# sjulier/Refactored_ORB_SLAM2

Hardware: AMD Instinct MI355X
Metric: frames/s (extract+match) at KITTI 1241×376, 2000 feat; 1/2/4/8 GPU + CPU ref (higher is better)
Workload: dtype u8; 1 GPU; kitti_stereo_1241x376_2000feat_8lvl: 2x ORBextractor + ComputeStereoMatches + SearchByProjection(cur,last); parallelism=frame-shard x1, collective=none, driver=torch, queries=one pass: orbfe_track_queries_stereo_device

## Files before the change

refactored_orb_slam2_amd/csrc/extract_kernels.hip:

```cpp
#include <stdlib.h>
#include <string.h>

#include "orbfe_internal.h"
#include "../../include/orb_pattern_data.h"

#define WAVE 64

__device__ __forceinline__ int wave_incl_scan(int v) {
  v += __builtin_amdgcn_update_dpp(0, v, 0x111, 0xf, 0xf, false);
  v += __builtin_amdgcn_update_dpp(0, v, 0x112, 0xf, 0xf, false);
  v += __builtin_amdgcn_update_dpp(0, v, 0x114, 0xf, 0xf, false);
  v += __builtin_amdgcn_update_dpp(0, v, 0x118, 0xf, 0xf, false);
  v += __builtin_amdgcn_update_dpp(0, v, 0x142, 0xa, 0xf, false);
  v += __builtin_amdgcn_update_dpp(0, v, 0x143, 0xc, 0xf, false);
  return v;
}

template <int T>
__device__ __forceinline__ int block_incl_scan_t(int v, int* tmp, int* total) {
  const int tid = threadIdx.x;
  const int lane = tid & (WAVE - 1), wid = tid >> 6;
  int s = wave_incl_scan(v);
  if (T == WAVE) {
    *total = __builtin_amdgcn_readlane(s, WAVE - 1);
    return s;
  }
  __syncthreads();
  if (lane == WAVE - 1) tmp[wid] = s;
  __syncthreads();
  int off = 0, tot = 0;
#pragma unroll
  for (int i = 0; i < T / WAVE; i++) {
    int t = tmp[i];
    if (i < wid) off += t;
    tot += t;
  }
  *total = tot;
  return s + off;
}

template <int T>
__device__ __forceinline__ int block_incl_scan_alt(int v, int* tmp, int& slot, int* total) {
  const int tid = threadIdx.x;
  const int lane = tid & (WAVE - 1), wid = tid >> 6;
  const int s = wave_incl_scan(v);
  int* t = tmp + slot * (T / WAVE);
  slot ^= 1;
  if (lane == WAVE - 1) t[wid] = s;
  __syncthreads();
  int off = 0, tot = 0;
#pragma unroll
  for (int i = 0; i < T / WAVE; i++) {
    const int x = t[i];
    if (i < wid) off += x;
    tot += x;
  }
  *total = tot;
  return s + off;
}

__device__ __forceinline__ int reflect101(int p, int len) {
  if (len == 1) return 0;
  while (p < 0 || p >= len) p = (p < 0) ? -p : 2 * (len - 1) - p;
  return p;
}

__global__ __launch_bounds__(256) void copy_level0_kernel(const uint8_t* __restrict__ src, int sstride,
                                                           unsigned long long simg, uint8_t* __restrict__ dst,
                                                           int dpitch, unsigned long long dimg, int w, int h, int tiled) {
  const int nchunk = (w + 15) >> 4;
  const int item = blockIdx.x * 256 + threadIdx.x;
  const int y = (int)((item + 0.5f) * (1.0f / (float)nchunk));
  const int x16 = (item - y * nchunk) * 16;
  if (y >= h) return;
  const uint8_t* S = src + (size_t)blockIdx.z * simg + (size_t)y * sstride;
  uint32_t out[4];
  if (x16 + 20 <= w) {
    const uintptr_t A = reinterpret_cast<uintptr_t>(S + x16);
    const uint32_t sh = (uint32_t)(A & 3);
    const uint32_t* B = reinterpret_cast<const uint32_t*>(A - sh);
    uint32_t d[5];
#pragma unroll
    for (int i = 0; i < 5; i++) d[i] = B[i];
#pragma unroll
// ... 1394 lines not shown
  hi = (int)__builtin_amdgcn_perm(t23, t01, 0x07060302u);
}
#ifndef BT_MFMA
#define BT_MFMA 1
#endif
#define BT_W 64
#define BT_H ORBFE_BLUR_TILE_H
#if BT_MFMA
#define BT_INP 96
#define BT_COL0 12
#else
#define BT_INP 80
#define BT_COL0 0
#endif
#define BT_HP 68
#ifndef BT_NT_STORE
#define BT_NT_STORE 1
#endif
#ifndef BT_NT_LOAD
#define BT_NT_LOAD 0
#endif
#ifndef BT_XCD_IMAGES
#define BT_XCD_IMAGES 1
#endif
#ifndef BT_SCALAR_TILE
#define BT_SCALAR_TILE 1
#endif
#ifndef BT_MIN_WAVES
#define BT_MIN_WAVES 2
#endif
#ifndef BT_THREADS
#define BT_THREADS 128
#endif
template <bool RESIZE, int THREADS>
__global__ __launch_bounds__(THREADS, BT_MIN_WAVES) void blur_level_kernel(PyrView src, PyrView dst, const BlurTile* __restrict__ tiles, int n_tiles,
                                                         LevelResize rz) {
#if BT_MFMA
  __shared__ __attribute__((aligned(16))) uint8_t in[65 * BT_INP];
#else
  __shared__ __attribute__((aligned(16))) uint8_t in[(BT_H + 6) * BT_INP];
  __shared__ __attribute__((aligned(16))) uint32_t hbp[((BT_H + 6) / 2) * BT_HP];
#endif
  const int tid = threadIdx.x;
#if BT_MFMA
  const int mlane = tid & 63, mwave = __builtin_amdgcn_readfirstlane(tid >> 6);
  const v4i* mtab = reinterpret_cast<const v4i*>(g_blur_tile_tab);
  const v4i HB = mtab[mlane];
#endif
#if BT_XCD_IMAGES
  int tile_id = (int)blockIdx.x, img = (int)blockIdx.y;
  {
    const unsigned gx = gridDim.x;
    const unsigned lin = blockIdx.y * gx + blockIdx.x;
    const unsigned grp = lin / (8u * gx);
    if (8u * grp + 8u <= gridDim.y) {
      const unsigned within = lin - grp * 8u * gx;
      img = (int)(8u * grp + (within & 7u));
      tile_id = (int)(within >> 3);
    }
  }
#else
  const int q = blockIdx.x >> 3, img = (int)blockIdx.y;
  const int tile_id = (int)blockIdx.x >= (n_tiles / 64) * 64 ? (int)blockIdx.x : (q >> 3) * 64 + (blockIdx.x & 7) * 8 + (q & 7);
#endif
#if BT_SCALAR_TILE
  static_assert(sizeof(BlurTile) == 16, "four dwords");
  BlurTile t;
  {
    const __attribute__((address_space(4))) uint32_t* q =
        (const __attribute__((address_space(4))) uint32_t*)(uintptr_t)(tiles + __builtin_amdgcn_readfirstlane(tile_id));
    uint32_t w4[4];
#pragma unroll
    for (int j = 0; j < 4; j++) w4[j] = q[j];
    __builtin_memcpy(&t, w4, sizeof(t));
  }
#else
  const BlurTile t = tiles[tile_id];
#endif
  const int lvl = t.level;
  const int w = src.w[lvl], h = src.h[lvl], pitch = src.pitch[lvl];
  const uint8_t* S = src.base[lvl] + (size_t)img * src.img_stride[lvl];
  uint8_t* D = const_cast<uint8_t*>(dst.base[lvl]) + (size_t)img * dst.img_stride[lvl];
  const int ox = t.tx * BT_W, oy = t.ty * BT_H;
  const bool stiled = (src.tiled >> lvl) & 1u;
  const int J = t.j0 + (tid & (ORBFE_FUSE_DWORDS - 1));
  __shared__ uint4 ytap[16 * ORBFE_FUSE_ROWS];
  __shared__ uint32_t ydst[16 * ORBFE_FUSE_ROWS];
  uint2 txr[4], tyl = make_uint2(0u, 0u);
  if constexpr (RESIZE) {
#pragma unroll
    for (int i = 0; i < 4; i++) txr[i] = reinterpret_cast<const uint2*>(rz.xt)[min(4 * J + i, rz.dw - 1)];
    tyl = reinterpret_cast<const uint2*>(rz.yt)[min(t.r0 + min(tid, 16 * ORBFE_FUSE_ROWS - 1), rz.dh - 1)];
  }
  {
    uint32_t* in32 = reinterpret_cast<uint32_t*>(in);
    constexpr int NC = RESIZE ? 19 : 18;
    constexpr int RPP = THREADS / NC, NLD = (BT_H + 6 + RPP - 1) / RPP;
    const int r0 = tid / NC, c = tid - r0 * NC;
    const int x = ox - 4 + 4 * c;
    uint32_t v[NLD];
    const bool interior = oy >= 3 && oy + BT_H + 3 <= h && ox >= 4 && ox - 4 + 4 * NC <= w;
    const bool tilepath = stiled && BT_COL0 != 0;
    if (r0 < RPP && !tilepath) {
      if (interior && stiled) {
        const uint32_t xoff = ((uint32_t)(x >> 4) << 7) + (uint32_t)(x & 15), tstep = (uint32_t)(pitch >> 4) << 7;
#pragma unroll
        for (int k = 0; k < NLD; k++) {
          const int y = oy - 3 + r0 + RPP * k;
          v[k] = r0 + RPP * k < BT_H + 6 ? *reinterpret_cast<const uint32_t*>(S + (uint32_t)(y >> 3) * tstep + (uint32_t)((y & 7) * 16) + xoff) : 0u;
        }
      } else if (interior) {
        const uint8_t* p0 = S + (size_t)(oy - 3 + r0) * pitch + x;
#pragma unroll
        for (int k = 0; k < NLD; k++)
#if BT_NT_LOAD
          v[k] = r0 + RPP * k < BT_H + 6 ? __builtin_nontemporal_load(reinterpret_cast<const uint32_t*>(p0 + (size_t)(RPP * k) * pitch)) : 0u;
#else
          v[k] = r0 + RPP * k < BT_H + 6 ? *reinterpret_cast<const uint32_t*>(p0 + (size_t)(RPP * k) * pitch) : 0u;
#endif
      } else {
        const bool whole = x >= 0 && x + 3 < w;
        int gx[4];
#pragma unroll
        for (int j = 0; j < 4; j++) gx[j] = reflect101(x + j, w);
#pragma unroll
        for (int k = 0; k < NLD; k++) {
          const int r = r0 + RPP * k;
          v[k] = 0u;
          if (r < BT_H + 6) {
            const int yy = reflect101(oy + r - 3, h);
            auto px = [&](int xx) { return (uint32_t)S[orbfe_level_offset(xx, yy, pitch, stiled)]; };
            if (whole) v[k] = *reinterpret_cast<const uint32_t*>(S + orbfe_level_offset(x, yy, pitch, stiled));
            else v[k] = px(gx[0]) | (px(gx[1]) << 8) | (px(gx[2]) << 16) | (px(gx[3]) << 24);
          }
        }
      }
#pragma unroll
      for (int k = 0; k < NLD; k++) {
        const int r = r0 + RPP * k;
        if (r < BT_H + 6) in32[r * (BT_INP / 4) + BT_COL0 / 4 + c] = v[k];
      }
    }
#if BT_MFMA
    if (tilepath) {
      constexpr int N_TOP = 3 * 6, N_MID = 7 * 8 * 6, N_ALL = N_TOP + N_MID + 3 * 6;
      constexpr int NP = (N_ALL + THREADS - 1) / THREADS;
      const int ty0 = (oy - 3) >> 3, tx0 = (ox - 16) >> 4;
      const int tiles_y = (h + 7) >> 3, tiles_x = pitch >> 4;
      const uint32_t tstep = (uint32_t)tiles_x << 7;
      auto piece = [&](int pid, int& tyi, int& txi, int& rr) {
        if (pid < N_TOP) { txi = (pid * 43) >> 7; rr = 5 + pid - 3 * txi; tyi = 0; }
        else if (pid < N_TOP + N_MID) { const int q = pid - N_TOP, tl = q >> 3; rr = q & 7; tyi = (tl * 43) >> 8; txi = tl - 6 * tyi; tyi += 1; }
        else { const int q = pid - N_TOP - N_MID; txi = (q * 43) >> 7; rr = q - 3 * txi; tyi = 8; }
      };
      uint4 pv[NP];
      uint32_t lds_at[NP];
#pragma unroll
      for (int k = 0; k < NP; k++) {
        int tyi, txi, rr;
        piece(min(tid + k * THREADS, N_ALL - 1), tyi, txi, rr);
        const int tr = min(max(ty0 + tyi, 0), tiles_y - 1), tc = min(max(tx0 + txi, 0), tiles_x - 1);
        pv[k] = *reinterpret_cast<const uint4*>(S + (uint32_t)tr * tstep + ((uint32_t)tc << 7) + (uint32_t)(rr * 16));
        lds_at[k] = (uint32_t)((tyi * 8 + rr - 5) * BT_INP + 16 * txi);
      }
#pragma unroll
      for (int k = 0; k < NP; k++)
        if (tid + k * THREADS < N_ALL) *reinterpret_cast<uint4*>(in + lds_at[k]) = pv[k];
      if (!interior) {
        __syncthreads();
        {
          const int nl = ox == 0 ? 3 : 0, nr = w < ox - 4 + 4 * NC ? 3 : 0;
          for (int i = tid; i < (BT_H + 6) * (nl + nr); i += THREADS) {
            const int wr = (int)((i + 0.5f) * (1.0f / (float)(nl + nr))), j = i - wr * (nl + nr);
            const int xx = j < nl ? j - 3 : w + (j - nl);
            const int y = oy - 3 + wr;
            if (y >= 0 && y < h && xx - (ox - 16) < BT_INP)
              in[wr * BT_INP + (xx - (ox - 16))] = in[wr * BT_INP + (reflect101(xx, w) - (ox - 16))];
          }
        }
        __syncthreads();
        {
          const int nt = oy == 0 ? 3 : 0, nb = h < oy + BT_H + 3 ? 3 : 0;
          for (int i = tid; i < (nt + nb) * (BT_INP / 4); i += THREADS) {
            const int j = (int)((i + 0.5f) * (1.0f / (float)(BT_INP / 4))), cdw = i - j * (BT_INP / 4);
            const int y = j < nt ? j - 3 : h + (j - nt);
            const int wr = y - (oy - 3), ws = reflect101(y, h) - (oy - 3);
            if (wr >= 0 && wr < BT_H + 6) in32[wr * (BT_INP / 4) + cdw] = in32[ws * (BT_INP / 4) + cdw];
          }
        }
      }
    }
#endif
  }
  if constexpr (RESIZE)
    if (tid < 16 * ORBFE_FUSE_ROWS) {
      const int ra = (int)(int16_t)(tyl.x & 0xffff) - (oy - 3), rb = (int)(int16_t)(tyl.x >> 16) - (oy - 3);
      ytap[tid] = make_uint4((uint32_t)(ra * BT_INP), (uint32_t)(rb * BT_INP), (tyl.y & 0xffffu) << 12, (tyl.y >> 16) << 12);
      const int yd = t.r0 + tid;
      ydst[tid] = rz.dst_tiled ? (uint32_t)(yd >> 3) * ((uint32_t)(rz.dpitch >> 4) << 7) + (uint32_t)((yd & 7) * 16) : (uint32_t)yd * (uint32_t)rz.dpitch;
    }
  __syncthreads();
  if constexpr (RESIZE) {
    typedef __attribute__((ext_vector_type(2))) unsigned short us2;
    if (J < t.j1) {
      const int s00 = (int)(int16_t)(txr[0].x & 0xffff);
      const int base = s00 - (ox - 4) + BT_COL0;
      const uint32_t sh = (uint32_t)base & 3u;
      uint32_t sel[4], cp[4];
#pragma unroll
      for (int i = 0; i < 4; i++) {
        const uint32_t o = (uint32_t)((int)(int16_t)(txr[i].x & 0xffff) - s00);
        sel[i] = o | 0x0c000c00u | ((o + 1) << 16);
        cp[i] = txr[i].y;
      }
      const uint32_t trow = (uint32_t)(uintptr_t)(in + (base & ~3));
      auto hrow2 = [&](uint32_t off_a, uint32_t off_b, uint32_t (&ha)[4], uint32_t (&hb)[4]) {
        unsigned long long a01, b01;
        uint32_t a2, b2;
        asm volatile("ds_read2_b32 %0, %4 offset1:1\n\t"
                     "ds_read_b32 %1, %4 offset:8\n\t"
                     "ds_read2_b32 %2, %5 offset1:1\n\t"
                     "ds_read_b32 %3, %5 offset:8\n\t"
                     "s_waitcnt lgkmcnt(0)"
                     : "=&v"(a01), "=&v"(a2), "=&v"(b01), "=&v"(b2)
                     : "v"(trow + off_a), "v"(trow + off_b)
                     : "memory");
        const uint32_t A0 = __builtin_amdgcn_alignbyte((uint32_t)(a01 >> 32), (uint32_t)a01, sh), A1 = __builtin_amdgcn_alignbyte(a2, (uint32_t)(a01 >> 32), sh);
        const uint32_t B0w = __builtin_amdgcn_alignbyte((uint32_t)(b01 >> 32), (uint32_t)b01, sh), B1w = __builtin_amdgcn_alignbyte(b2, (uint32_t)(b01 >> 32), sh);
#pragma unroll
        for (int i = 0; i < 4; i++) {
          const uint32_t ua = __builtin_amdgcn_perm(A1, A0, sel[i]), ub = __builtin_amdgcn_perm(B1w, B0w, sel[i]);
          ha[i] = __builtin_amdgcn_udot2(__builtin_bit_cast(us2, ua), __builtin_bit_cast(us2, cp[i]), 0u, false) & ~15u;
          hb[i] = __builtin_amdgcn_udot2(__builtin_bit_cast(us2, ub), __builtin_bit_cast(us2, cp[i]), 0u, false) & ~15u;
        }
      };
      uint8_t* Nimg = rz.dst + (size_t)img * rz.dimg;
      const uint32_t ncol = rz.dst_tiled ? (((uint32_t)((4 * J) >> 4) << 7) + (uint32_t)((4 * J) & 15)) : (uint32_t)(4 * J);
      for (int yi = tid >> 4; yi < t.r1 - t.r0; yi += THREADS / 16) {
        uint8_t* N = Nimg + (ncol + ydst[yi]);
        {
          const uint4 ty = ytap[yi];
          uint32_t h0[4], h1[4];
          hrow2(ty.x, ty.y, h0, h1);
          const uint32_t B0 = ty.z, B1 = ty.w;
          uint32_t sm[4];
#pragma unroll
          for (int i = 0; i < 4; i++) sm[i] = mulhi_u24(B0, h0[i]) + mulhi_u24(B1, h1[i]) + 2u;
          const uint32_t P01 = (sm[0] | (sm[1] << 16)) >> 2, P23 = (sm[2] | (sm[3] << 16)) >> 2;
          *reinterpret_cast<uint32_t*>(N) = __builtin_amdgcn_perm(P23, P01, 0x06040200u);
        }
      }
    }
  }
#if BT_MFMA
  {
    const int q = mlane >> 4, r = mlane & 15;
    const v4i c128 = {128, 128, 128, 128}, zero = {0, 0, 0, 0};
    const v4i cfin = {8388608 + 32768, 8388608 + 32768, 8388608 + 32768, 8388608 + 32768};
    v4i TB[4];
#pragma unroll
    for (int b = 0; b < 4; b++) TB[b] = mtab[(1 + b) * 64 + mlane];
    const uint32_t bstep = (uint32_t)(dst.pitch[lvl] >> 4) << 8;
#pragma unroll
    for (int g = mwave; g < BT_W / 16; g += THREADS / 64) {
      v4i Xh, Xl;
      {
        const v4i* arow = reinterpret_cast<const v4i*>(in + r * BT_INP + 16 * g + 16 * q);
        v4i A[4];
#pragma unroll
        for (int blk = 0; blk < 4; blk++) A[blk] = arow[blk * BT_INP];
        int ph[4], pl[4];
#pragma unroll
        for (int blk = 0; blk < 4; blk++) {
          const v4i d = __builtin_amdgcn_mfma_i32_16x16x64_i8(A[blk] ^ (int)0x80808080, HB, c128, 0, 0, 0);
          blur_pack(d, ph[blk], pl[blk]);
        }
        Xh = v4i{ph[0], ph[1], ph[2], ph[3]};
        Xl = v4i{pl[0], pl[1], pl[2], pl[3]};
      }
      const int gx = ox + 16 * g + 4 * q;
      uint8_t* o = D + blur_tiled_offset(gx, oy + r, dst.pitch[lvl]);
#pragma unroll
      for (int b = 0; b < 4; b++) {
        const v4i vh = __builtin_amdgcn_mfma_i32_16x16x64_i8(Xh, TB[b], zero, 0, 0, 0);
        const v4i vl = __builtin_amdgcn_mfma_i32_16x16x64_i8(Xl, TB[b], cfin, 0, 0, 0);
        const uint32_t r0 = ((uint32_t)vh.x << 8) + (uint32_t)vl.x, r1 = ((uint32_t)vh.y << 8) + (uint32_t)vl.y;
        const uint32_t r2 = ((uint32_t)vh.z << 8) + (uint32_t)vl.z, r3 = ((uint32_t)vh.w << 8) + (uint32_t)vl.w;
        const uint32_t out = __builtin_amdgcn_perm(r1, r0, 0x0c0c0602u) | __builtin_amdgcn_perm(r3, r2, 0x06020c0cu);
        const int row = 16 * b + r;
        if (gx < w && row < BT_H && oy + row < h) {
#if BT_NT_STORE
          __builtin_nontemporal_store(out, reinterpret_cast<uint32_t*>(o + b * bstep));
#else
          *reinterpret_cast<uint32_t*>(o + b * bstep) = out;
#endif
        }
      }
    }
  }
}
#else
  for (int it = tid; it < ((BT_H + 6) / 2) * 16; it += THREADS) {
    const int k = it >> 4, g = it & 15;
    uint32_t o[2][4];
#pragma unroll
    for (int rr = 0; rr < 2; rr++) {
      const uint32_t* p = reinterpret_cast<const uint32_t*>(in + (2 * k + rr) * BT_INP + 4 * g);
      const uint32_t w0 = p[0], w1 = p[1], w2 = p[2];
#define TAPS(a, b, c, d) ((uint32_t)(a) | ((uint32_t)(b) << 8) | ((uint32_t)(c) << 16) | ((uint32_t)(d) << 24))
#define DOT4(x, t, acc) __builtin_amdgcn_udot4((x), (t), (acc), false)
      o[rr][0] = DOT4(w1, TAPS(56, 48, 34, 18), DOT4(w0, TAPS(0, 18, 34, 48), 0u));
      o[rr][1] = DOT4(w2, TAPS(18, 0, 0, 0), DOT4(w1, TAPS(48, 56, 48, 34), DOT4(w0, TAPS(0, 0, 18, 34), 0u)));
      o[rr][2] = DOT4(w2, TAPS(34, 18, 0, 0), DOT4(w1, TAPS(34, 48, 56, 48), DOT4(w0, TAPS(0, 0, 0, 18), 0u)));
      o[rr][3] = DOT4(w2, TAPS(48, 34, 18, 0), DOT4(w1, TAPS(18, 34, 48, 56), 0u));
#undef DOT4
#undef TAPS
    }
    uint4 st;
    st.x = o[0][0] | (o[1][0] << 16);
    st.y = o[0][1] | (o[1][1] << 16);
    st.z = o[0][2] | (o[1][2] << 16);
    st.w = o[0][3] | (o[1][3] << 16);
    *reinterpret_cast<uint4*>(hbp + k * BT_HP + 4 * g) = st;
  }
  __syncthreads();
  {
    typedef __attribute__((ext_vector_type(2))) unsigned short us2;
    for (int it = tid; it < (BT_H / 2) * 16; it += THREADS) {
    const int g = it & 15, rp = it >> 4;
    uint4 P[4];
#pragma unroll
    for (int k = 0; k < 4; k++) P[k] = *reinterpret_cast<const uint4*>(hbp + (rp + k) * BT_HP + 4 * g);
    const uint32_t E0 = 18u | (34u << 16), E1 = 48u | (56u << 16), E2 = 48u | (34u << 16), E3 = 18u;
    const uint32_t O0 = 18u << 16, O1 = 34u | (48u << 16), O2 = 56u | (48u << 16), O3 = 34u | (18u << 16);
    uint32_t aE[4], aO[4];
#pragma unroll
    for (int i = 0; i < 4; i++) {
      const uint32_t p0 = i == 0 ? P[0].x : i == 1 ? P[0].y : i == 2 ? P[0].z : P[0].w;
      const uint32_t p1 = i == 0 ? P[1].x : i == 1 ? P[1].y : i == 2 ? P[1].z : P[1].w;
      const uint32_t p2 = i == 0 ? P[2].x : i == 1 ? P[2].y : i == 2 ? P[2].z : P[2].w;
      const uint32_t p3 = i == 0 ? P[3].x : i == 1 ? P[3].y : i == 2 ? P[3].z : P[3].w;
#define UD2(a, b, c) __builtin_amdgcn_udot2(__builtin_bit_cast(us2, (uint32_t)(a)), __builtin_bit_cast(us2, (uint32_t)(b)), (c), false)
      const uint32_t accE = UD2(p3, E3, UD2(p2, E2, UD2(p1, E1, UD2(p0, E0, 32768u))));
      const uint32_t accO = UD2(p3, O3, UD2(p2, O2, UD2(p1, O1, UD2(p0, O0, 32768u))));
#undef UD2
      aE[i] = accE;
      aO[i] = accO;
    }
    const uint32_t outE = __builtin_amdgcn_perm(aE[1], aE[0], 0x0c0c0602u) | __builtin_amdgcn_perm(aE[3], aE[2], 0x06020c0cu);
    const uint32_t outO = __builtin_amdgcn_perm(aO[1], aO[0], 0x0c0c0602u) | __builtin_amdgcn_perm(aO[3], aO[2], 0x06020c0cu);
    const int gy = oy + 2 * rp, gx = ox + 4 * g;
    if (gx < w) {
      uint8_t* o = D + blur_tiled_offset(gx, gy, dst.pitch[lvl]);
#if BT_NT_STORE
      if (gy < h) __builtin_nontemporal_store(outE, reinterpret_cast<uint32_t*>(o));
      if (gy + 1 < h) __builtin_nontemporal_store(outO, reinterpret_cast<uint32_t*>(o + 16));
#else
      if (gy < h) *reinterpret_cast<uint32_t*>(o) = outE;
      if (gy + 1 < h) *reinterpret_cast<uint32_t*>(o + 16) = outO;
#endif
    }
    }
  }
}
#endif

#ifndef BLUR_RING
#define BLUR_RING 2
#endif
#ifndef BLUR_MIN_BLOCKS
#define BLUR_MIN_BLOCKS 4
#endif
#define BLUR_DMA(gsrc, lds_dst) do { \
    unsigned keep_m0; \
    asm volatile("s_mov_b32 %0, m0\n\ts_mov_b32 m0, %2\n\ts_nop 0\n\tglobal_load_lds_dwordx4 %1, off\n\ts_mov_b32 m0, %0" \
                 : "=&s"(keep_m0) : "v"(gsrc), "s"(lds_dst) : "memory"); \
  } while (0)
#if BLUR_RING == 2
#define BLUR_WAIT_ROWS() asm volatile("s_waitcnt vmcnt(6)" ::: "memory")
#elif BLUR_RING == 3
#define BLUR_WAIT_ROWS() asm volatile("s_waitcnt vmcnt(14)" ::: "memory")
// ... 832 lines not shown
```

refactored_orb_slam2_amd/csrc/extractor.cpp:

```cpp
#include <math.h>
#include <stdarg.h>
#include <stdio.h>
#include <stdlib.h>
#include <string.h>

#include <algorithm>
#include <atomic>
#include <mutex>
#include <vector>

#include "host_internal.h"
#include "orbfe_internal.h"

void orbfe_launch_copy0(const uint8_t* src, int sstride, size_t simg, uint8_t* dst, int dpitch, size_t dimg, int w,
                        int h, int n_images, int tiled, hipStream_t s);
int orbfe_set_octree_lds(size_t lds_bytes);
int orbfe_upload_pattern_floats();

static thread_local char g_err[512] = "";
void orbfe_set_error(const char* fmt, ...) {
  va_list ap;
  va_start(ap, fmt);
  vsnprintf(g_err, sizeof(g_err), fmt, ap);
  va_end(ap);
// ... 328 lines not shown
    o.kp_off = kp_off;
    kp_off += o.kp_cap;
    maxM = std::max(maxM, o.kp_cap);
    o.key_off = key_off;
    o.key_cap = (int)std::min<size_t>(level_slots, 0xFFFFFF);
    key_off += level_slots;
  }
  for (CellDesc& c : e->cells) {
    const int tw = std::max(c.cols - 6, 0), th = std::max(c.rows - 6, 0);
    const int ppr = std::max((tw + 1) >> 1, 1), ri = std::max(64 / ppr, 1);
    c.ppr = (int16_t)ppr; c.ri = (int16_t)ri; c.n_it = (int16_t)((th + ri - 1) / ri);
    c.inv_ppr = 1.0f / (float)ppr;
  }
  std::vector<ResizeTap> hxt[ORBFE_MAX_LEVELS], hyt[ORBFE_MAX_LEVELS];
  for (int l = 1; l < nl; l++) {
    std::vector<ResizeTap>&xt = hxt[l], &yt = hyt[l];
    build_taps(e->lg[l - 1].w, e->lg[l].w, true, xt);
    build_taps(e->lg[l - 1].h, e->lg[l].h, false, yt);
    bool ok = true;
    for (int x0 = 0; x0 < (int)xt.size() && ok; x0 += 256) {
      const int xl = std::min<int>(x0 + 255, (int)xt.size() - 1);
      const int sxa = xt[x0].s0 & ~15;
      if ((((xt[xl].s1 - sxa) >> 4) + 1) * 16 > 560) ok = false;
    }
    for (int y0 = 0; y0 < (int)yt.size() && ok; y0 += 16) {
      const int yl = std::min<int>(y0 + 15, (int)yt.size() - 1);
      if (yt[yl].s1 - yt[y0].s0 + 1 > 34) ok = false;
    }
    bool win8 = ok;
    for (int y0 = 0; y0 < (int)yt.size() && win8; y0 += 32) {
      const int yl = std::min<int>(y0 + 31, (int)yt.size() - 1);
      if (yt[yl].s1 - yt[y0].s0 + 1 > 42) win8 = false;
    }
    for (int x4 = 0; x4 < (int)xt.size() && win8; x4 += 4) {
      const int xe = std::min<int>(x4 + 3, (int)xt.size() - 1);
      if (xt[xe].s0 + 1 - xt[x4].s0 > 7) win8 = false;
      for (int i = x4; i <= xe; i++)
        if (xt[i].c1 != 0 && xt[i].s1 != xt[i].s0 + 1) win8 = false;
    }
    bool narrow = win8;
    for (int x0 = 0; x0 < (int)xt.size() && narrow; x0 += 256) {
      const int xl = std::min<int>(x0 + 255, (int)xt.size() - 1);
      if (((xt[xl].s1 - (xt[x0].s0 & ~15)) >> 4) + 1 > 21) narrow = false;
    }
    e->resize_mode[l] = narrow ? 3 : win8 ? 2 : ok ? 1 : 0;
  }
  for (int l = 0; l < nl; l++) {
    const LevelGeom& g = e->lg[l];
    const int tiles_x = (g.w + 63) / 64, tiles_y = (g.h + ORBFE_BLUR_TILE_H - 1) / ORBFE_BLUR_TILE_H;
    std::vector<int> jx(tiles_x + 1, 0), ry(tiles_y + 1, 0);
    bool fuse = l + 1 < nl && e->resize_mode[l + 1] >= 2;
    if (fuse) {
      const std::vector<ResizeTap>&xt = hxt[l + 1], &yt = hyt[l + 1];
      const int dw = (int)xt.size(), dh = (int)yt.size(), ndw = (dw + 3) / 4;
      for (int tx = 0, j = 0; tx <= tiles_x; tx++) {
        while (j < ndw && xt[4 * j].s0 < 64 * tx) j++;
        jx[tx] = tx == tiles_x ? ndw : j;
      }
      for (int ty = 0, y = 0; ty <= tiles_y; ty++) {
        while (y < dh && yt[y].s0 < ORBFE_BLUR_TILE_H * ty) y++;
        ry[ty] = ty == tiles_y ? dh : y;
      }
      for (int tx = 0; tx < tiles_x && fuse; tx++) {
        if (jx[tx + 1] - jx[tx] > ORBFE_FUSE_DWORDS) fuse = false;
        for (int j = jx[tx]; j < jx[tx + 1] && fuse; j++) {
          const int xe = std::min(4 * j + 3, dw - 1);
          if (xt[4 * j].s0 < 64 * tx || xt[xe].s0 + 1 > 64 * tx + 71) fuse = false;
        }
      }
      for (int ty = 0; ty < tiles_y && fuse; ty++) {
        if (ry[ty + 1] - ry[ty] > 16 * ORBFE_FUSE_ROWS) fuse = false;
        for (int y = ry[ty]; y < ry[ty + 1] && fuse; y++)
          if (yt[y].s0 < ORBFE_BLUR_TILE_H * ty || yt[y].s1 > ORBFE_BLUR_TILE_H * ty + ORBFE_BLUR_TILE_H + 2) fuse = false;
      }
    }
    e->fuse_ok[l] = fuse;
    e->tile_first[l] = (int)e->tiles.size();
    for (int ty = 0; ty < tiles_y; ty++)
      for (int tx = 0; tx < tiles_x; tx++) {
        BlurTile bt;
        memset(&bt, 0, sizeof(bt));
        bt.level = (int16_t)l; bt.tx = (int16_t)tx; bt.ty = (int16_t)ty;
        if (fuse) { bt.j0 = (int16_t)jx[tx]; bt.j1 = (int16_t)jx[tx + 1]; bt.r0 = (int16_t)ry[ty]; bt.r1 = (int16_t)ry[ty + 1]; }
        e->tiles.push_back(bt);
      }
    e->tile_count[l] = (int)e->tiles.size() - e->tile_first[l];
  }
  e->blur_mfma = build_blur_tables(e);
  e->total_cells = (int)e->cells.size();
  e->slots_per_image = slot_off;
  e->gkeys_per_image = key_off;
  e->kp_per_image = kp_off;
  e->max_nodes = (maxM + 63) & ~63;
  if (e->max_nodes > 8192) {
    orbfe_set_error("nFeatures too large for the octree node table (%d nodes)", e->max_nodes);
    return ORBFE_ERR_INVALID;
  }
  {
    const size_t fixed = orbfe_octree_lds_bytes(e->max_nodes, 0);
    const size_t budget = 40 * 1024;
    e->lds_keys = fixed + 8 * 512 <= budget ? (int)((budget - fixed) / 8) : 512;
    e->oct_lds = orbfe_octree_lds_bytes(e->max_nodes, e->lds_keys);
    for (int l = 0; l < e->prm.n_levels; l++) {
      OctLevel& o = e->oct[l];
      o.ff_depth = 0;
      for (int D = 1; D <= 5; D++) {
        const size_t cells = (size_t)o.n_ini << (2 * D);
        const size_t counts = (size_t)o.n_ini * (((size_t)1 << (2 * D + 2)) - 4) / 3;
        const size_t need = counts * 4 + ((cells + 1) & ~(size_t)1) * 2 + (size_t)e->max_nodes * 4;
        if (cells <= 4096 && need <= (size_t)e->lds_keys * 8) o.ff_depth = D;
      }
    }
    if (e->oct_lds > 160 * 1024) {
      orbfe_set_error("octree LDS %zu exceeds 160 KiB", e->oct_lds);
      return ORBFE_ERR_INVALID;
    }
    if (e->oct_lds > 64 * 1024) {
      int rc = orbfe_set_octree_lds(e->oct_lds);
      if (rc != 0) {
        orbfe_set_error("hipFuncSetAttribute(max dynamic LDS %zu) failed: %d", e->oct_lds, rc);
        return ORBFE_ERR_HIP;
      }
    }
  }
  int rc;
  if ((rc = upload(e->d_cells, e->cells.data(), e->cells.size() * sizeof(CellDesc), e->stream))) return rc;
  if ((rc = upload(e->d_groups, e->groups.data(), e->groups.size() * sizeof(FastGroup), e->stream))) return rc;
  {
    std::vector<FastGroup> g1(e->cells.size());
    for (size_t i = 0; i < e->cells.size(); i++) {
      memset(&g1[i], 0, sizeof(FastGroup));
      g1[i].first_cell = (int32_t)i;
      g1[i].n_cells = 1;
      g1[i].level = e->cells[i].level;
    }
    if ((rc = upload(e->d_groups1, g1.data(), g1.size() * sizeof(FastGroup), e->stream))) return rc;
    HIPCHK(hipStreamSynchronize(e->stream));
  }
  if ((rc = upload(e->d_tiles, e->tiles.data(), e->tiles.size() * sizeof(BlurTile), e->stream))) return rc;
  if ((rc = upload(e->d_strips, e->strips.data(), e->strips.size() * sizeof(BlurStrip), e->stream))) return rc;
  if ((rc = upload(e->d_blur_tab, e->blur_tab.data(), e->blur_tab.size(), e->stream))) return rc;
  for (int l = 1; l < nl; l++) {
    if ((rc = upload(e->d_xt[l], hxt[l].data(), hxt[l].size() * sizeof(ResizeTap), e->stream))) return rc;
    if ((rc = upload(e->d_yt[l], hyt[l].data(), hyt[l].size() * sizeof(ResizeTap), e->stream))) return rc;
  }
  HIPCHK(hipStreamSynchronize(e->stream));
  e->plan_w = w;
  e->plan_h = h;
  e->cap_images = 0;
  return ORBFE_OK;
}

static size_t pyr_bytes_per_image(const orbfe_extractor* e) {
  size_t s = 0;
  for (int l = 0; l < e->prm.n_levels; l++) s += e->lg[l].plane;
  return s;
}

static int ensure_workspace(orbfe_extractor* e, int n_images) {
  if (n_images <= e->cap_images) return ORBFE_OK;
  HIPCHK(hipStreamSynchronize(e->stream));
  const size_t B = (size_t)n_images;
  int rc;
  if ((rc = dev_alloc(e->d_pyr, pyr_bytes_per_image(e) * B + 4096))) return rc;
  if ((rc = dev_alloc(e->d_blur, pyr_bytes_per_image(e) * B + 4096))) return rc;
  if ((rc = dev_alloc(e->d_cell_cnt, sizeof(int32_t) * e->total_cells * B))) return rc;
// ... 763 lines not shown
```

refactored_orb_slam2_amd/csrc/orbfe_internal.h:

```cpp
#pragma once
#include <hip/hip_runtime.h>
#include <stdint.h>

#include "../../include/orbfe.h"

#define ORBFE_EDGE 16
#define ORBFE_CELL_MAX 66
#ifndef ORBFE_BLUR_TILE_H
#define ORBFE_BLUR_TILE_H 56
#endif
#define ORBFE_MAX_INI 256
#ifndef ORBFE_OCT_THREADS
#define ORBFE_OCT_THREADS 256
#endif

struct PyrView {
  const uint8_t* base[ORBFE_MAX_LEVELS];
  unsigned long long img_stride[ORBFE_MAX_LEVELS];
  int pitch[ORBFE_MAX_LEVELS];
  int w[ORBFE_MAX_LEVELS], h[ORBFE_MAX_LEVELS];
  int n_levels;
  unsigned tiled;
};

// ... 4 lines not shown
  return (((uint32_t)(y >> 3) * (uint32_t)(pitch >> 4) + (uint32_t)(x >> 4)) << 7) + (uint32_t)((y & 7) * 16 + (x & 15));
}
__host__ __device__ inline uint32_t orbfe_level_offset(int x, int y, int pitch, bool tiled) {
  return tiled ? orbfe_tiled_offset(x, y, pitch) : (uint32_t)y * (uint32_t)pitch + (uint32_t)x;
}

struct ResizeTap {
  int16_t s0, s1;
  int16_t c0, c1;
};

struct CellDesc {
  int16_t level;
  int16_t x0, y0;
  int16_t cols, rows;
  int16_t shift_x, shift_y;
  int16_t slot_cap;
  uint32_t slot_off;
  int16_t ppr, ri, n_it, pad;
  float inv_ppr;
};

#ifndef ORBFE_FG_MAX
#define ORBFE_FG_MAX 4
#define ORBFE_FG_MAX_WIDTH 176
#endif
struct FastGroup {
  int32_t first_cell;
  int16_t n_cells, level;
  int16_t x0, y0, width, rows;
  int16_t wcell, pad;
};

struct OctLevel {
  int cell_begin, n_cells;
  int N;
  int n_ini;
  float hX;
  int width, height;
  int kp_off, kp_cap;
  unsigned long long key_off;
  int key_cap;
  int ff_depth;
};

struct OctParams {
  OctLevel lv[ORBFE_MAX_LEVELS];
  const CellDesc* cells;
  const int32_t* cell_cnt;
  const uint32_t* slots;
  int32_t* cell_off;
  unsigned long long* gkeys;
  uint32_t* lvl_kp;
  int32_t* lvl_n;
  int32_t* err;
  int total_cells;
  unsigned long long slots_per_image, gkeys_per_image;
  int kp_per_image;
  int n_levels;
  int max_nodes;
  int lds_keys;
};

struct DescribeParams {
  PyrView pyr;
  PyrView blur;
  const uint32_t* lvl_kp;
  const int32_t* lvl_n;
  int kp_off[ORBFE_MAX_LEVELS], kp_cap[ORBFE_MAX_LEVELS];
  float scale[ORBFE_MAX_LEVELS];
  float kp_size[ORBFE_MAX_LEVELS];
  int kp_per_image;
  int n_levels;
  orbfe_keypoint* out_kps;
  uint8_t* out_desc;
  int32_t* out_n;
  int cap;
  int xcd_images;
};

struct BlurTile {
  int16_t level, tx, ty;
  int16_t j0, j1, r0, r1;
  int16_t pad;
};
struct LevelResize {
  uint8_t* dst;
  unsigned long long dimg;
  int dpitch, dw, dh;
  int dst_tiled;
  const ResizeTap* xt;
  const ResizeTap* yt;
};
#define ORBFE_FUSE_DWORDS 16
#define ORBFE_FUSE_ROWS 3

#define ORBFE_BLUR_CHUNK 48
#define ORBFE_BLUR_WINDOW 32
struct BlurStrip {
  int16_t level, chunk;
};
struct BlurMfmaParams {
  const BlurStrip* strips;
  int n_strips;
  const uint8_t* tab;
  uint32_t b_off[ORBFE_MAX_LEVELS];
  uint32_t t_off;
  int use;
};

void orbfe_launch_resize(const uint8_t* src, int spitch, size_t simg, uint8_t* dst, int dpitch, size_t dimg, int dw,
                         int dh, const ResizeTap* xt, const ResizeTap* yt, int n_images, int mode, hipStream_t s);
void orbfe_launch_fast_cells(const PyrView& pyr, const CellDesc* cells, const FastGroup* groups, int n_groups, int total_cells,
                             int cell_rows, int cell_span, int sc_max, int bits_max, int32_t* cell_cnt, uint32_t* slots,
                             unsigned long long slots_per_image, int ini_th, int min_th, int n_images, hipStream_t s);
void orbfe_launch_octree(const OctParams& p, int n_images, size_t lds_bytes, hipStream_t s);
void orbfe_launch_blur(const PyrView& src, const PyrView& dst, const BlurTile* tiles, int n_tiles, const BlurMfmaParams& mf,
                       int n_images, hipStream_t s);
void orbfe_launch_blur_level(const PyrView& src, const PyrView& dst, const BlurTile* tiles, int n_tiles, const LevelResize* rz,
                             int n_images, hipStream_t s);
void orbfe_launch_describe(const DescribeParams& p, int n_images, hipStream_t s);
size_t orbfe_octree_lds_bytes(int max_nodes, int lds_keys);
```

Measured before the change: 113,300 frames/s.

## Precompute blur tile edge info to skip partial-tile MFMA work and simplify borders

Host-side tile setup now packs per-tile metadata (valid column groups, vertical/horizontal block counts, and edge flags) into the former pad field of BlurTile. The MFMA blur kernel uses this to skip out-of-image tile loads, MFMA passes and stores on partial edge tiles. It also replaces per-pixel reflect101 gathers with clamped dword loads followed by an LDS border fix-up. The full-tile case is kept as a separate template instance so interior tiles stay branch-free. The border rewrite adds hand-coded reflection logic that must match the old behaviour at every image edge, which is a correctness risk.

```diff
diff --git a/refactored_orb_slam2_amd/csrc/extract_kernels.hip b/refactored_orb_slam2_amd/csrc/extract_kernels.hip
--- a/refactored_orb_slam2_amd/csrc/extract_kernels.hip
+++ b/refactored_orb_slam2_amd/csrc/extract_kernels.hip
@@ -1,5 +1,6 @@
 #include <stdlib.h>
 #include <string.h>
+#include <type_traits>
 
 #include "orbfe_internal.h"
 #include "../../include/orb_pattern_data.h"
@@ -1560,6 +1561,7 @@
   const uint8_t* S = src.base[lvl] + (size_t)img * src.img_stride[lvl];
   uint8_t* D = const_cast<uint8_t*>(dst.base[lvl]) + (size_t)img * dst.img_stride[lvl];
   const int ox = t.tx * BT_W, oy = t.ty * BT_H;
+  const uint32_t tinfo = t.info;
   const bool stiled = (src.tiled >> lvl) & 1u;
   const int J = t.j0 + (tid & (ORBFE_FUSE_DWORDS - 1));
   __shared__ uint4 ytap[16 * ORBFE_FUSE_ROWS];
@@ -1577,7 +1579,11 @@
     const int r0 = tid / NC, c = tid - r0 * NC;
     const int x = ox - 4 + 4 * c;
     uint32_t v[NLD];
+#if BT_MFMA
+    const bool interior = (tinfo & ORBFE_BT_EDGES) == 0;
+#else
     const bool interior = oy >= 3 && oy + BT_H + 3 <= h && ox >= 4 && ox - 4 + 4 * NC <= w;
+#endif
     const bool tilepath = stiled && BT_COL0 != 0;
     if (r0 < RPP && !tilepath) {
       if (interior && stiled) {
@@ -1597,6 +1603,14 @@
           v[k] = r0 + RPP * k < BT_H + 6 ? *reinterpret_cast<const uint32_t*>(p0 + (size_t)(RPP * k) * pitch) : 0u;
 #endif
       } else {
+#if BT_MFMA
+        const uint8_t* p0 = S + min(max(x, 0), ((w + 3) & ~3) - 4);
+#pragma unroll
+        for (int k = 0; k < NLD; k++) {
+          const int r = r0 + RPP * k;
+          v[k] = r < BT_H + 6 ? *reinterpret_cast<const uint32_t*>(p0 + (uint32_t)min(max(oy - 3 + r, 0), h - 1) * (uint32_t)pitch) : 0u;
+        }
+#else
         const bool whole = x >= 0 && x + 3 < w;
         int gx[4];
 #pragma unroll
@@ -1612,6 +1626,7 @@
             else v[k] = px(gx[0]) | (px(gx[1]) << 8) | (px(gx[2]) << 16) | (px(gx[3]) << 24);
           }
         }
+#endif
       }
 #pragma unroll
       for (int k = 0; k < NLD; k++) {
@@ -1631,39 +1646,65 @@
         else if (pid < N_TOP + N_MID) { const int q = pid - N_TOP, tl = q >> 3; rr = q & 7; tyi = (tl * 43) >> 8; txi = tl - 6 * tyi; tyi += 1; }
         else { const int q = pid - N_TOP - N_MID; txi = (q * 43) >> 7; rr = q - 3 * txi; tyi = 8; }
       };
-      uint4 pv[NP];
-      uint32_t lds_at[NP];
-#pragma unroll
-      for (int k = 0; k < NP; k++) {
-        int tyi, txi, rr;
-        piece(min(tid + k * THREADS, N_ALL - 1), tyi, txi, rr);
-        const int tr = min(max(ty0 + tyi, 0), tiles_y - 1), tc = min(max(tx0 + txi, 0), tiles_x - 1);
-        pv[k] = *reinterpret_cast<const uint4*>(S + (uint32_t)tr * tstep + ((uint32_t)tc << 7) + (uint32_t)(rr * 16));
-        lds_at[k] = (uint32_t)((tyi * 8 + rr - 5) * BT_INP + 16 * txi);
-      }
-#pragma unroll
-      for (int k = 0; k < NP; k++)
-        if (tid + k * THREADS < N_ALL) *reinterpret_cast<uint4*>(in + lds_at[k]) = pv[k];
-      if (!interior) {
-        __syncthreads();
-        {
-          const int nl = ox == 0 ? 3 : 0, nr = w < ox - 4 + 4 * NC ? 3 : 0;
-          for (int i = tid; i < (BT_H + 6) * (nl + nr); i += THREADS) {
-            const int wr = (int)((i + 0.5f) * (1.0f / (float)(nl + nr))), j = i - wr * (nl + nr);
-            const int xx = j < nl ? j - 3 : w + (j - nl);
-            const int y = oy - 3 + wr;
-            if (y >= 0 && y < h && xx - (ox - 16) < BT_INP)
-              in[wr * BT_INP + (xx - (ox - 16))] = in[wr * BT_INP + (reflect101(xx, w) - (ox - 16))];
-          }
-        }
-        __syncthreads();
-        {
-          const int nt = oy == 0 ? 3 : 0, nb = h < oy + BT_H + 3 ? 3 : 0;
-          for (int i = tid; i < (nt + nb) * (BT_INP / 4); i += THREADS) {
-            const int j = (int)((i + 0.5f) * (1.0f / (float)(BT_INP / 4))), cdw = i - j * (BT_INP / 4);
-            const int y = j < nt ? j - 3 : h + (j - nt);
-            const int wr = y - (oy - 3), ws = reflect101(y, h) - (oy - 3);
-            if (wr >= 0 && wr < BT_H + 6) in32[wr * (BT_INP / 4) + cdw] = in32[ws * (BT_INP / 4) + cdw];
+      auto stage = [&](auto bottom) {
+        constexpr bool BOTTOM = decltype(bottom)::value;
+        const int wr_last = min(h - oy + 5, BT_H + 5);
+        bool need[NP];
+#pragma unroll
+        for (int k = 0; k < NP; k++) {
+          const int p0 = mwave * 64 + k * THREADS;
+          const int first = p0 < N_TOP ? 0 : p0 < N_TOP + N_MID ? 8 * ((((p0 - N_TOP) >> 3) * 43) >> 8) + 3 : BT_H + 3;
+          need[k] = !BOTTOM || first <= wr_last;
+        }
+        uint4 pv[NP];
+        uint32_t lds_at[NP];
+#pragma unroll
+        for (int k = 0; k < NP; k++) {
+          int tyi, txi, rr;
+          piece(min(tid + k * THREADS, N_ALL - 1), tyi, txi, rr);
+          const int tr = min(max(ty0 + tyi, 0), tiles_y - 1), tc = min(max(tx0 + txi, 0), tiles_x - 1);
+          if constexpr (BOTTOM) pv[k] = make_uint4(0u, 0u, 0u, 0u);
+          if (need[k]) pv[k] = *reinterpret_cast<const uint4*>(S + (uint32_t)tr * tstep + ((uint32_t)tc << 7) + (uint32_t)(rr * 16));
+          lds_at[k] = (uint32_t)((tyi * 8 + rr - 5) * BT_INP + 16 * txi);
+        }
+#pragma unroll
+        for (int k = 0; k < NP; k++)
+          if (need[k] && tid + k * THREADS < N_ALL) *reinterpret_cast<uint4*>(in + lds_at[k]) = pv[k];
+      };
+      if (tinfo & ORBFE_BT_BOTTOM) stage(std::true_type{});
+      else stage(std::false_type{});
+    }
+    if (!interior) {
+      __syncthreads();
+      auto refl = [](int p, int len) {
+        int r = p < 0 ? -p : p >= len ? 2 * len - 2 - p : p;
+        if ((unsigned)r >= (unsigned)len) r = reflect101(p, len);
+        return r;
+      };
+      const int wr_hi = (tinfo & ORBFE_BT_BOTTOM) ? min(h - oy + 5, BT_H + 5) : BT_H + 5;
+      if (tinfo & (ORBFE_BT_LEFT | ORBFE_BT_RIGHT)) {
+        const int nl = (tinfo & ORBFE_BT_LEFT) ? 3 : 0, nr = (tinfo & ORBFE_BT_RIGHT) ? 3 : 0;
+        for (int i = tid; i < 64 * (nl + nr); i += THREADS) {
+          const int j = i >> 6, wr = i & 63;
+          const int xx = j < nl ? j - 3 : w + (j - nl);
+          if (wr <= wr_hi)
+            in[wr * BT_INP + (xx - (ox - 16))] = in[(refl(oy - 3 + wr, h) - (oy - 3)) * BT_INP + (refl(xx, w) - (ox - 16))];
+        }
+      }
+      if (tinfo & (ORBFE_BT_TOP | ORBFE_BT_BOTTOM)) {
+        const int nt = (tinfo & ORBFE_BT_TOP) ? 3 : 0, nb = (tinfo & ORBFE_BT_BOTTOM) ? 3 : 0;
+        const int xs = (tinfo & ORBFE_BT_RIGHT) ? (w & ~3) : w;
+        for (int i = tid; i < 32 * (nt + nb); i += THREADS) {
+          const int j = i >> 5, cdw = i & 31;
+          const int y = j < nt ? j - 3 : h + (j - nt);
+          const int wr = y - (oy - 3), ws = refl(y, h) - (oy - 3);
+          const int xx = ox - 16 + 4 * cdw, xb = xs + (cdw - BT_INP / 4);
+          if (wr <= BT_H + 5) {
+            if (cdw < BT_INP / 4) {
+              if (xx >= 0 && xx + 3 < w) in32[wr * (BT_INP / 4) + cdw] = in32[ws * (BT_INP / 4) + cdw];
+            } else if (xb < w) {
+              in[wr * BT_INP + (xb - (ox - 16))] = in[ws * BT_INP + (xb - (ox - 16))];
+            }
           }
         }
       }
@@ -1739,27 +1780,39 @@
 #pragma unroll
     for (int b = 0; b < 4; b++) TB[b] = mtab[(1 + b) * 64 + mlane];
     const uint32_t bstep = (uint32_t)(dst.pitch[lvl] >> 4) << 8;
+    auto blur_part = [&](auto full) {
+    constexpr bool FULL = decltype(full)::value;
+    const int n_groups = ORBFE_BT_GROUPS(tinfo), n_vblocks = ORBFE_BT_VBLOCKS(tinfo), n_hblocks = ORBFE_BT_HBLOCKS(tinfo);
 #pragma unroll
     for (int g = mwave; g < BT_W / 16; g += THREADS / 64) {
+      if (!FULL && g >= n_groups) continue;
       v4i Xh, Xl;
       {
         const v4i* arow = reinterpret_cast<const v4i*>(in + r * BT_INP + 16 * g + 16 * q);
-        v4i A[4];
-#pragma unroll
-        for (int blk = 0; blk < 4; blk++) A[blk] = arow[blk * BT_INP];
-        int ph[4], pl[4];
-#pragma unroll
-        for (int blk = 0; blk < 4; blk++) {
-          const v4i d = __builtin_amdgcn_mfma_i32_16x16x64_i8(A[blk] ^ (int)0x80808080, HB, c128, 0, 0, 0);
-          blur_pack(d, ph[blk], pl[blk]);
-        }
-        Xh = v4i{ph[0], ph[1], ph[2], ph[3]};
-        Xl = v4i{pl[0], pl[1], pl[2], pl[3]};
+        auto hpass = [&](auto nh) {
+          constexpr int NH = decltype(nh)::value;
+          v4i A[4];
+#pragma unroll
+          for (int blk = 0; blk < NH; blk++) A[blk] = arow[blk * BT_INP];
+          int ph[4] = {0, 0, 0, 0}, pl[4] = {0, 0, 0, 0};
+#pragma unroll
+          for (int blk = 0; blk < NH; blk++) {
+            const v4i d = __builtin_amdgcn_mfma_i32_16x16x64_i8(A[blk] ^ (int)0x80808080, HB, c128, 0, 0, 0);
+            blur_pack(d, ph[blk], pl[blk]);
+          }
+          Xh = v4i{ph[0], ph[1], ph[2], ph[3]};
+          Xl = v4i{pl[0], pl[1], pl[2], pl[3]};
+        };
+        if (FULL || n_hblocks >= 4) hpass(std::integral_constant<int, 4>{});
+        else if (n_hblocks == 3) hpass(std::integral_constant<int, 3>{});
+        else if (n_hblocks == 2) hpass(std::integral_constant<int, 2>{});
+        else hpass(std::integral_constant<int, 1>{});
       }
       const int gx = ox + 16 * g + 4 * q;
       uint8_t* o = D + blur_tiled_offset(gx, oy + r, dst.pitch[lvl]);
 #pragma unroll
       for (int b = 0; b < 4; b++) {
+        if (!FULL && b >= n_vblocks) continue;
         const v4i vh = __builtin_amdgcn_mfma_i32_16x16x64_i8(Xh, TB[b], zero, 0, 0, 0);
         const v4i vl = __builtin_amdgcn_mfma_i32_16x16x64_i8(Xl, TB[b], cfin, 0, 0, 0);
         const uint32_t r0 = ((uint32_t)vh.x << 8) + (uint32_t)vl.x, r1 = ((uint32_t)vh.y << 8) + (uint32_t)vl.y;
@@ -1775,6 +1828,9 @@
         }
       }
     }
+    };
+    if ((tinfo & 0x1ffu) == (4u | 4u << 3 | 4u << 6)) blur_part(std::true_type{});
+    else blur_part(std::false_type{});
   }
 }
 #else
diff --git a/refactored_orb_slam2_amd/csrc/extractor.cpp b/refactored_orb_slam2_amd/csrc/extractor.cpp
--- a/refactored_orb_slam2_amd/csrc/extractor.cpp
+++ b/refactored_orb_slam2_amd/csrc/extractor.cpp
@@ -434,6 +434,7 @@
         memset(&bt, 0, sizeof(bt));
         bt.level = (int16_t)l; bt.tx = (int16_t)tx; bt.ty = (int16_t)ty;
         if (fuse) { bt.j0 = (int16_t)jx[tx]; bt.j1 = (int16_t)jx[tx + 1]; bt.r0 = (int16_t)ry[ty]; bt.r1 = (int16_t)ry[ty + 1]; }
+        bt.info = orbfe_blur_tile_info(g.w, g.h, tx, ty);
         e->tiles.push_back(bt);
       }
     e->tile_count[l] = (int)e->tiles.size() - e->tile_first[l];
diff --git a/refactored_orb_slam2_amd/csrc/orbfe_internal.h b/refactored_orb_slam2_amd/csrc/orbfe_internal.h
--- a/refactored_orb_slam2_amd/csrc/orbfe_internal.h
+++ b/refactored_orb_slam2_amd/csrc/orbfe_internal.h
@@ -110,8 +110,26 @@
 struct BlurTile {
   int16_t level, tx, ty;
   int16_t j0, j1, r0, r1;
-  int16_t pad;
+  uint16_t info;
 };
+#define ORBFE_BT_GROUPS(i) ((int)((i) & 7u))
+#define ORBFE_BT_VBLOCKS(i) ((int)(((i) >> 3) & 7u))
+#define ORBFE_BT_HBLOCKS(i) ((int)(((i) >> 6) & 7u))
+#define ORBFE_BT_LEFT 0x0200u
+#define ORBFE_BT_RIGHT 0x0400u
+#define ORBFE_BT_TOP 0x0800u
+#define ORBFE_BT_BOTTOM 0x1000u
+#define ORBFE_BT_EDGES 0x1e00u
+inline uint16_t orbfe_blur_tile_info(int w, int h, int tx, int ty) {
+  const int ox = tx * 64, oy = ty * ORBFE_BLUR_TILE_H;
+  const int cols = w - ox < 64 ? w - ox : 64, rows = h - oy < ORBFE_BLUR_TILE_H ? h - oy : ORBFE_BLUR_TILE_H;
+  unsigned i = (unsigned)((cols + 15) / 16) | (unsigned)((rows + 15) / 16) << 3 | (unsigned)((rows + 6 + 15) / 16) << 6;
+  if (tx == 0) i |= ORBFE_BT_LEFT;
+  if (w < ox + 72) i |= ORBFE_BT_RIGHT;
+  if (ty == 0) i |= ORBFE_BT_TOP;
+  if (h < oy + ORBFE_BLUR_TILE_H + 3) i |= ORBFE_BT_BOTTOM;
+  return (uint16_t)i;
+}
 struct LevelResize {
   uint8_t* dst;
   unsigned long long dimg;
```

Measured after the change: 114,100 frames/s, median of 6. Within noise of the previous version (+0.7%).
